# AnteMarusic/Accelerating-Genomics

Measured on AMD Instinct MI355X. Metric: Smith-Waterman affine-gap score-only GCUPS (config 2: 65536 pairs 150x150 per GPU), higher is better.
Workload: dtype int16x2 lanes, int32 scores; 1 GPU; BASELINE config 2: 65536 SW pairs 150x150 per GPU, iid ACGT + 25% related, newline sentinel aligned as the reference does; pairs_per_gpu=65536, len=150, cells_counted_per_pair=22500, parallelism=pairs sharded per GPU, no collective

## Files before the change

accelerating-genomics_amd/api.py:

```python
from __future__ import annotations

import ctypes as C
import os
import subprocess

import numpy as np

_HERE = os.path.dirname(os.path.abspath(__file__))
TUNING_KNOBS = ("AGX_SW_KERNEL", "AGX_SW_TAIL_BETA", "AGX_SW_MAX_C", "AGX_SW_FORCE_C", "AGX_SW_MAX_CLASSES", "AGX_SW_WAVES_PER_CLASS",
                "AGX_SW_SORT_WAVES", "AGX_SW_ONE_LAUNCH", "AGX_SW_DNA", "AGX_SW_RISE", "AGX_PHMM_PLAIN_CELL", "AGX_TRACE_CREATE", "AGX_HOST_THREADS", "AGX_FANOUT", "AGX_PHMM_TAB_BUDGET", "AGX_PHMM_MAX_C",
                "AGX_PHMM_FORCE_C", "AGX_PHMM_TAIL_BETA", "AGX_PHMM_MAX_CLASSES", "AGX_PHMM_NO_LUT", "AGX_TRACE_POOL", "AGX_NO_STREAM_PRIO", "AGX_SW_I32_CLASSIC", "AGX_SW_PIECE_MB", "AGX_SW_PIECE_MIN_PAIRS", "AGX_PHMM_NO_ROWS", "AGX_PHMM_NO_TRAINS", "AGX_PHMM_LUT_ONE_LOOP", "AGX_SW_HOST_PLAN", "AGX_PHMM_NO_RING")
_DEFAULT_LIB = "libagx_tuning.so" if any(k in os.environ for k in TUNING_KNOBS) else "libagx.so"
LIB_PATH = os.environ.get("AGX_LIB_PATH", os.path.join(_HERE, _DEFAULT_LIB))

OK, E_ARG, E_NODEVICE, E_HIP, E_NOMEM, E_SYMBOL, E_LIMIT, E_IO = 0, -1, -2, -3, -4, -5, -6, -7
OPT_SW_KERNEL = 1
OPT_SW_PLANNER = 2
SW_PLANNER_AUTO, SW_PLANNER_HOST, SW_PLANNER_DEVICE = 0, 1, 2
OPT_PHMM_TRAINS = 3
PHMM_TRAINS_AUTO, PHMM_TRAINS_OFF, PHMM_TRAINS_ON = 0, 1, 2
SW_KERNEL_AUTO, SW_KERNEL_INT32, SW_KERNEL_PACKED_SIGNED, SW_KERNEL_PACKED_BIASED = 0, 1, 2, 3
PHMM_F64, PHMM_F64_FMA, PHMM_F32, PHMM_F32_FMA = 0, 1, 2, 3
PHMM_GATK_PRIOR = 0x100

SYMBOLS = [
    "agx_version", "agx_last_error", "agx_device_count", "agx_device_name", "agx_ctx_create", "agx_ctx_destroy", "agx_ctx_device",
    "agx_ctx_stream", "agx_ctx_set_stream", "agx_ctx_sync", "agx_ctx_set_option", "agx_warmup_devices", "agx_host_alloc", "agx_host_free",
    "agx_ctx_timer_start", "agx_ctx_timer_stop", "agx_ctx_timer_mark", "agx_ctx_timer_elapsed",
    "agx_sw_batch_create", "agx_sw_batch_create_scored", "agx_sw_batch_create_matrix", "agx_sw_batch_launch", "agx_sw_batch_scores", "agx_sw_batch_bind_scores", "agx_sw_batch_info", "agx_sw_batch_destroy",
    "agx_sw_score", "agx_sw_score_multi", "agx_sw_score_devices", "agx_sw_shard_cuts",
    "agx_phmm_batch_create", "agx_phmm_batch_launch", "agx_phmm_batch_results", "agx_phmm_batch_bind_results", "agx_phmm_batch_info",
    "agx_phmm_batch_destroy", "agx_phmm_forward", "agx_phmm_forward_multi", "agx_phmm_forward_devices", "agx_phmm_shard_cuts",
    "agx_pairHMM",
    "agx_sw_text_read", "agx_sw_text_free", "agx_sw_reader_open", "agx_sw_reader_line_num", "agx_sw_reader_set_threads", "agx_sw_reader_next",
# ... 438 lines not shown
```

accelerating-genomics_amd/csrc/agx_sw.cpp:

```cpp
#include "agx_sw.h"

#include <algorithm>
#include <cmath>
#include <memory>
#include <mutex>
#include <thread>

#include "agx_internal.h"
#include "agx_parallel.h"

namespace {

struct Tiling {
    int cls;
    int G;
};

bool positive(long n) { return n > 0; }
bool at_least_4(long n) { return n >= 4; }
inline double tail_beta_override() { static const double v = agx_knob_real(agx_tune("AGX_SW_TAIL_BETA"), -1.0); return v; }
int max_cols_per_lane() { static const int v = (int)agx_knob_int(agx_tune("AGX_SW_MAX_C"), AGX_SW_MAX_COLS_PER_LANE, at_least_4); return v; }
int force_cols_per_lane() { static const int v = (int)agx_knob_int(agx_tune("AGX_SW_FORCE_C"), 0); return v; }
int max_classes_override() { static const int v = (int)agx_knob_int(agx_tune("AGX_SW_MAX_CLASSES"), 0, positive); return v; }
int tuned_kernel()
// ... 118 lines not shown
            best_cost = c;
        }
    }
    return best;
}

inline uint64_t piece_bytes() { static const uint64_t v = (uint64_t)agx_knob_int(agx_tune("AGX_SW_PIECE_MB"), 32, positive) << 20; return v; }
inline int64_t piece_min_pairs() { static const int64_t v = agx_knob_int(agx_tune("AGX_SW_PIECE_MIN_PAIRS"), 32768, positive); return v; }
constexpr size_t kRawPad = 64;
constexpr uint8_t kClsEmpty = 255;
constexpr uint8_t kClsUntiled = 254;
struct PairPlan {
    uint32_t pair;
    uint32_t ly;
    uint16_t lxo;
    uint8_t cls;
    uint8_t G;
    uint32_t lx() const { return lxo & 0x7fffu; }
};

struct ClassLaunch {
    int C = 0;
    uint32_t first_wave = 0, n_waves = 0;
};

struct Bucket {
    size_t first = 0, count = 0;
    size_t group0 = 0, n_groups = 0;
    size_t wave0 = 0, n_waves = 0;
    int cls = 0, G = 0;
};

}

struct agx_sw_batch {
    agx_ctx *ctx = nullptr;
    int family = 0;
    SwParams prm{};
    int64_t n_pairs = 0;
    DevBuf img, groups, waves, scores;
    DevBuf table;
    int rising = 0;
    PinBuf out_stage;
    bool matrix = false;
    std::vector<ClassLaunch> launches;
    agx_sw_info info{};
    struct SwPending *pending = nullptr;
// ... 903 lines not shown
        const char *e = agx_tune("AGX_SW_SORT_WAVES");
        return !(e && e[0] == '0');
    }();
    static const bool one_launch_ok = [] {
        const char *e = agx_tune("AGX_SW_ONE_LAUNCH");
        return !(e && e[0] == '0');
    }();
    if (family >= 2 && launches.size() > 1 && one_launch_ok) {
        if (sort_waves)
            std::stable_sort(waves.begin(), waves.end(), [](const SwWave &a, const SwWave &b) {
                return (uint64_t)a.steps * a.reserved > (uint64_t)b.steps * b.reserved;
            });
        ClassLaunch all_classes;
        all_classes.C = 0;
        all_classes.first_wave = 0;
        all_classes.n_waves = (uint32_t)waves.size();
        launches.assign(1, all_classes);
    } else if (sort_waves && !launches.empty())
        agx_pool_run((int)launches.size(), [&](int k) {
            const ClassLaunch &cl = launches[(size_t)k];
            std::stable_sort(waves.begin() + cl.first_wave, waves.begin() + cl.first_wave + cl.n_waves,
                             [](const SwWave &a, const SwWave &b) { return a.steps > b.steps; });
        });
    std::vector<uint32_t> x_dw(plan.size()), y_dw(plan.size());
    img_dw = img0;
    {
        const int parts = (int)std::min<int64_t>(agx_host_threads(), std::max<int64_t>(1, (int64_t)plan.size() / 16384));
        std::vector<size_t> part_sum((size_t)parts + 1, 0);
        const size_t chunk = (plan.size() + parts - 1) / (size_t)parts;
        auto words = [&](const PairPlan &pp, size_t *xw) {
            *xw = ((size_t)pp.G * kSwClasses[pp.cls] + 3) / 4 + 1;
            return *xw + ((size_t)pp.ly + 3) / 4;
        };
        agx_pool_run(parts, [&](int t) {
            const size_t lo = std::min(plan.size(), (size_t)t * chunk), hi = std::min(plan.size(), lo + chunk);
            size_t s = 0, xw;
            for (size_t i = lo; i < hi; ++i) s += words(plan[i], &xw);
            part_sum[(size_t)t + 1] = s;
        });
        for (int t = 0; t < parts; ++t) part_sum[(size_t)t + 1] += part_sum[(size_t)t];
        img_dw = img0 + part_sum[(size_t)parts];
        if (img_dw > 0xffffffffull) {
            agx_set_error("packed image exceeds 16 GiB; split the batch");
            return AGX_E_LIMIT;
        }
        agx_pool_run(parts, [&](int t) {
// ... 132 lines not shown
        agx_set_error("agx_sw_batch_create: upload -> %s", hipGetErrorString(e));
        return AGX_E_HIP;
    }
    if (device_plan) b->info.padded_cells = (int64_t) * (const unsigned long long *)dp.h_padded.p;
    if (flag[0]) {
        if (matrix)
            agx_set_error("pair %u contains a byte outside the substitution matrix's alphabet", flag[1]);
        else
            agx_set_error("pair %u contains byte 0x00, which is reserved as the padding symbol", flag[1]);
        return AGX_E_SYMBOL;
    }
    if (trace)
        fprintf(stderr,
                "[agx_sw_batch_create] %lld pairs%s: pass A %.2f ms | tiling %.2f, sort %.2f, waves %.2f, records %.2f | waited %.2f ms more "
                "for the upload of %.1f MB | device pack + sync %.2f ms\n",
                (long long)n_pairs, device_plan ? " (planned on the device)" : "", t_pass_a - t_begin, t_plan - t_pass_a, t_sort - t_plan, t_waves - t_sort, t_records - t_waves,
                t_joined - t_records, raw_bytes / 1e6, agx_now_ms() - t_joined);
    *out = b;
    b = nullptr;
    done.ok = true;
    return AGX_OK;
}

}

extern "C" {

int agx_sw_batch_launch(agx_sw_batch *b)
{
    if (!b) {
        agx_set_error("agx_sw_batch_launch: null batch");
        return AGX_E_ARG;
    }
    if (!b->ctx) {
        agx_set_error("this batch was planned without a context (no device): it cannot be launched");
        return AGX_E_NODEVICE;
    }
    int rc = agx_bind(b->ctx);
    if (rc) return rc;
    if (b->pending && b->pending->ready) AGX_HIP(hipStreamWaitEvent(b->ctx->stream, b->pending->ready, 0));
    SwParams prm = b->prm;
    if (b->bound) prm.n_out = (uint32_t)b->n_pairs;
    FanOut fan(b->ctx, (int)b->launches.size());
    rc = fan.begin();
    if (rc) return rc;
    int k = 0;
    for (auto it = b->launches.rbegin(); it != b->launches.rend(); ++it) {
        const ClassLaunch &cl = *it;
        hipStream_t st = fan.stream(k++);
        const uint32_t *img = (const uint32_t *)b->img.p;
        const SwWave *wv = (const SwWave *)b->waves.p + cl.first_wave;
        int32_t *scores = b->bound ? b->bound : (int32_t *)b->scores.p;
        int r;
        if (b->matrix)
            r = agx_sw_mat_launch_class(cl.C, prm, img, (const SwGroup *)b->groups.p, wv, cl.n_waves, scores,
                                        (const int16_t *)b->table.p, st);
        else if (b->family == 3)
            r = cl.C == 0 ? agx_sw_i32d_launch_any(prm, img, (const SwGroup2 *)b->groups.p, wv, cl.n_waves, scores, st)
                          : agx_sw_i32d_launch_class(cl.C, prm, img, (const SwGroup2 *)b->groups.p, wv, cl.n_waves, scores, st);
        else if (b->family == 2 && cl.C == 0)
            r = agx_sw_pk2_launch_any(b->rising, prm, img, (const SwGroup2 *)b->groups.p, wv, cl.n_waves, scores, st);
        else if (b->family == 2)
            r = agx_sw_pk2_launch_class(cl.C, b->rising, prm, img, (const SwGroup2 *)b->groups.p, wv, cl.n_waves, scores, st);
        else if (b->family == 1)
            r = agx_sw_pk_launch_class(cl.C, prm, img, (const SwGroup2 *)b->groups.p, wv, cl.n_waves, scores, st);
        else
            r = (cl.C > 40 ? agx_sw_wide_launch_class : agx_sw_launch_class)(cl.C, prm, img, (const SwGroup *)b->groups.p, wv,
                                                                             cl.n_waves, scores, st);
        if (r) {
            agx_set_error("sw_fill<%d> launch failed: %s", cl.C, hipGetErrorString(hipGetLastError()));
            return AGX_E_HIP;
        }
    }
    return fan.end();
}

int agx_sw_batch_scores(agx_sw_batch *b, int32_t *scores)
{
    if (!b || (!scores && b->n_pairs)) {
        agx_set_error("agx_sw_batch_scores: null argument");
        return AGX_E_ARG;
    }
    if (!b->ctx) {
        agx_set_error("this batch was planned without a context (no device): it has no scores");
        return AGX_E_NODEVICE;
    }
    int rc = agx_bind(b->ctx);
    if (rc) return rc;
    if (b->pending) {
        rc = finish_create(b);
        if (rc) return rc;
    }
    if (b->n_pairs == 0) {
        AGX_HIP(hipStreamSynchronize(b->ctx->stream));
        return AGX_OK;
    }
    const size_t bytes = (size_t)b->n_pairs * sizeof(int32_t);
    if (b->bound && scores == b->bound) {
        AGX_HIP(hipStreamSynchronize(b->ctx->stream));
        return AGX_OK;
    }
// ... 145 lines not shown
```

accelerating-genomics_amd/csrc/agx_sw.h:

```cpp
#pragma once
#include <hip/hip_runtime.h>

#include <algorithm>
#include <cstdint>

struct SwGroup {
    uint32_t x_dw;
    uint32_t y_dw;
    uint32_t lx_ly;
    uint32_t out;
};

struct SwParams {
    int32_t ge;
    int32_t gf;
    int32_t hd;
    int32_t delta;
    int32_t shift;
    uint32_t ge2, gf2, hd2, delta2;
    uint32_t age2, agf2, bias2;
    uint32_t n_out;
};

struct SwGroup2 {
    uint32_t x_dw[2];
    uint32_t y_dw[2];
    uint32_t lx_ly[2];
    uint32_t out[2];
};

struct SwWave {
    uint32_t first_group;
    uint16_t n_groups;
    uint16_t G;
    uint32_t steps;
    uint32_t reserved;
};

#define AGX_SW_FOR_EACH_CLASS(X) \
    X(4) X(6) X(8) X(10) X(12) X(14) X(16) X(18) X(20) X(22) X(24) X(26) X(28) X(30) X(32) X(34) X(36) X(38) X(40)
#define AGX_SW_FOR_EACH_WIDE_CLASS(X) X(80) X(120) X(160)
static const int kSwClasses[] = {4, 6, 8, 10, 12, 14, 16, 18, 20, 22, 24, 26, 28, 30, 32, 34, 36, 38, 40, 80, 120, 160};
static const int kSwPackedMaxShort = 64 * 40;
static const int kSwNumClasses = sizeof(kSwClasses) / sizeof(kSwClasses[0]);
static const double kSwClassCost[] = {1.373, 1.250, 1.178, 1.138, 1.112, 1.080, 1.051, 1.033, 1.025, 1.022, 1.014, 1.014, 1.011, 1.007, 1.007, 1.004, 1.004, 1.004, 1.000, 1.6, 2.2, 4.0};
static const double kSwPkClassCost[] = {1.543, 1.358, 1.278, 1.210, 1.173, 1.136, 1.111, 1.086, 1.068, 1.037, 1.025, 1.025, 1.019, 1.012, 1.006, 1.006, 1.006, 1.000, 1.000, 0, 0, 0};
static const double kSwPk2ClassCost[] = {1.851, 1.581, 1.450, 1.367, 1.318, 1.263, 1.196, 1.184, 1.145, 1.097, 1.095, 1.056, 1.049, 1.053, 1.025, 1.023, 1.022, 1.016, 1.000, 0, 0, 0};

static const double kSwI32dClassCost[] = {1.373, 1.250, 1.178, 1.138, 1.112, 1.080, 1.051, 1.033, 1.025, 1.022, 1.014, 1.014, 1.011, 1.007, 1.007, 1.004, 1.004, 1.004, 1.000, 0, 0, 0};

constexpr int kSwMatDim = 33;
int agx_sw_mat_launch_class(int cols_per_lane, const SwParams &prm, const uint32_t *img, const SwGroup *groups,
                            const SwWave *waves, uint32_t n_waves, int32_t *scores, const int16_t *table, hipStream_t s);
int agx_sw_pack_launch(bool matrix, int slots, const uint8_t *raw, const uint64_t *off, uint64_t base, const void *groups,
                       uint32_t n_groups, uint32_t n_pairs, uint32_t *img, const uint8_t *code, uint32_t *flag, int n_cu,
                       hipStream_t s);
int agx_sw_pack_dna_launch(const uint8_t *raw, const uint64_t *off, uint64_t base, void *groups, void *waves, uint32_t n_waves,
                           uint32_t n_pairs, uint32_t *img, uint32_t *flag, int n_cu, hipStream_t s);
int agx_sw_pk_launch_class(int cols_per_lane, const SwParams &prm, const uint32_t *img, const SwGroup2 *groups,
                           const SwWave *waves, uint32_t n_waves, int32_t *scores, hipStream_t s);
int agx_sw_pk2_launch_class(int cols_per_lane, int rising, const SwParams &prm, const uint32_t *img, const SwGroup2 *groups,
                            const SwWave *waves, uint32_t n_waves, int32_t *scores, hipStream_t s);
void agx_sw_pk2_preload();
void agx_sw_pack_preload();
void agx_sw_i32_preload();
int agx_sw_pk2_launch_any(int rising, const SwParams &prm, const uint32_t *img, const SwGroup2 *groups, const SwWave *waves, uint32_t n_waves,
                          int32_t *scores, hipStream_t s);
int agx_sw_i32d_launch_any(const SwParams &prm, const uint32_t *img, const SwGroup2 *groups, const SwWave *waves, uint32_t n_waves, int32_t *scores,
                           hipStream_t s);
int agx_sw_i32d_launch_class(int cols_per_lane, const SwParams &prm, const uint32_t *img, const SwGroup2 *groups, const SwWave *waves,
                             uint32_t n_waves, int32_t *scores, hipStream_t s);
void agx_sw_i32d_preload();
int agx_sw_launch_class(int cols_per_lane, const SwParams &prm, const uint32_t *img, const SwGroup *groups,
                        const SwWave *waves, uint32_t n_waves, int32_t *scores, hipStream_t s);
int agx_sw_wide_launch_class(int cols_per_lane, const SwParams &prm, const uint32_t *img, const SwGroup *groups,
                             const SwWave *waves, uint32_t n_waves, int32_t *scores, hipStream_t s);

constexpr uint32_t kSwPlanEmptyKey = 1u << 27;
constexpr uint32_t kSwPlanWaveKeyMax = (1u << 24) - 1u;
constexpr int kSwPlanBuckets = kSwNumClasses * 64;
struct SwPlanArgs {
    const uint32_t *len;
    uint32_t n_pairs, n_fill;
    const uint32_t *seg_first;
    const uint32_t *segs;
// ... 18 lines not shown
```

accelerating-genomics_amd/csrc/agx_sw_pk2_kernel.hip:

```cpp
#include "agx_sw.h"
#include <type_traits>

namespace {

typedef unsigned short u16x2 __attribute__((ext_vector_type(2)));

__device__ __forceinline__ u16x2 as_v(uint32_t v) { return __builtin_bit_cast(u16x2, v); }
__device__ __forceinline__ uint32_t as_u(u16x2 v) { return __builtin_bit_cast(uint32_t, v); }
__device__ __forceinline__ uint32_t umax2(uint32_t a, uint32_t b) { return as_u(__builtin_elementwise_max(as_v(a), as_v(b))); }
__device__ __forceinline__ uint32_t umin2(uint32_t a, uint32_t b) { return as_u(__builtin_elementwise_min(as_v(a), as_v(b))); }
typedef _Float16 f16x2 __attribute__((ext_vector_type(2)));
__device__ __forceinline__ uint32_t umax3(uint32_t a, uint32_t b, uint32_t c)
{
    const f16x2 x = __builtin_bit_cast(f16x2, a), y = __builtin_bit_cast(f16x2, b), z = __builtin_bit_cast(f16x2, c);
    return __builtin_bit_cast(uint32_t, __builtin_elementwise_maximum(__builtin_elementwise_maximum(x, y), z));
}
__device__ __forceinline__ uint32_t in_vgpr(uint32_t s)
{
    uint32_t r;
    asm volatile("v_mov_b32 %0, %1" : "=v"(r) : "s"(s));
    return r;
}

#define AGX_DPP_TAKE " wave_shr:1 row_mask:0xf bank_mask:0xf bound_ctrl:0\n"

#define AGX_FAST_HEAD(BYTE)                                                                                                  \
    asm("v_lshrrev_b32_sdwa %4, %6, %8 dst_sel:DWORD dst_unused:UNUSED_PAD src0_sel:" BYTE " src1_sel:DWORD\n"               \
        "v_lshrrev_b32_sdwa %5, %7, %8 dst_sel:DWORD dst_unused:UNUSED_PAD src0_sel:" BYTE " src1_sel:DWORD\n"               \
        "s_mov_b64 vcc, %9\n"                                                                                                \
        "v_cndmask_b32_dpp %0, %10, %12, vcc" AGX_DPP_TAKE "v_cndmask_b32_dpp %1, %11, %12, vcc" AGX_DPP_TAKE                \
        "v_cndmask_b32_dpp %2, %2, %4, vcc" AGX_DPP_TAKE "v_cndmask_b32_dpp %3, %3, %5, vcc" AGX_DPP_TAKE                    \
        : "=&v"(zl), "=&v"(fl), "+v"(ta), "+v"(tb), "=&v"(ma), "=&v"(mb)                                                     \
        : "v"(rowsA), "v"(rowsB), "v"(kv), "s"(start_mask), "v"(z_last), "v"(f_last), "v"(z0v)                               \
        : "vcc")

template <int K>
__device__ __forceinline__ void fast_head(uint32_t &zl, uint32_t &fl, uint32_t &ta, uint32_t &tb, uint32_t rowsA, uint32_t rowsB,
                                          uint32_t kv, uint64_t start_mask, uint32_t z_last, uint32_t f_last, uint32_t z0v)
{
    uint32_t ma, mb;
    if constexpr (K == 1)
        AGX_FAST_HEAD("BYTE_1");
    else if constexpr (K == 2)
        AGX_FAST_HEAD("BYTE_2");
    else if constexpr (K == 3)
        AGX_FAST_HEAD("BYTE_3");
    else
        AGX_FAST_HEAD("BYTE_0");
}

__device__ __forceinline__ void bytes_head(uint32_t &zl, uint32_t &fl, uint32_t &yc, uint32_t rowsA, uint32_t rowsB, uint32_t sel,
                                           uint32_t sh_sym, uint64_t start_mask, uint32_t z_last, uint32_t f_last, uint32_t z0v)
{
    uint32_t fresh;
    asm("v_perm_b32 %3, %5, %4, %6\n"
        "v_lshlrev_b32 %3, %7, %3\n"
        "s_mov_b64 vcc, %8\n"
        "v_cndmask_b32_dpp %0, %9, %11, vcc" AGX_DPP_TAKE "v_cndmask_b32_dpp %1, %10, %11, vcc" AGX_DPP_TAKE
        "v_cndmask_b32_dpp %2, %2, %3, vcc" AGX_DPP_TAKE
        : "=&v"(zl), "=&v"(fl), "+v"(yc), "=&v"(fresh)
        : "v"(rowsA), "v"(rowsB), "s"(sel), "v"(sh_sym), "s"(start_mask), "v"(z_last), "v"(f_last), "v"(z0v)
        : "vcc");
}

template <int C, bool FAST, int KC>
__device__ __forceinline__ void pk2_fill(const SwParams &prm, const uint32_t *__restrict__ img, const SwGroup2 &g, const SwWave &w,
                                         int32_t *__restrict__ scores, int lane, int G, int gl, bool active, bool start, bool feeder)
{
    constexpr int XW = (C + 3) / 4;
    constexpr bool RISE = KC > 0;
    constexpr int NK = KC > 1 ? KC : 1;
    constexpr int kEnd = KC > 1 ? (C - 1) % KC : 0;
    constexpr int NM = KC > 1 ? KC + 3 : NK;
    const uint32_t sh_sym = prm.shift;
    const uint32_t col_pad = 0x100u << sh_sym;
    const uint32_t ge = in_vgpr(prm.age2), gf = in_vgpr(RISE ? prm.agf2 - prm.age2 : prm.agf2);
    const uint32_t hd = in_vgpr(FAST ? prm.hd2 - prm.delta2 : prm.hd2);
    const uint32_t bias = prm.bias2, delta = prm.delta2;
    const uint32_t z0 = prm.bias2 - prm.agf2;
    const uint32_t hd0 = in_vgpr((FAST ? prm.hd2 - prm.delta2 : prm.hd2) + (RISE ? prm.age2 : 0u));
    const uint32_t hdw = in_vgpr((FAST ? prm.hd2 - prm.delta2 : prm.hd2) + prm.age2 - (uint32_t)NK * prm.age2);
    const uint32_t ge_wrap = in_vgpr((uint32_t)NK * prm.age2), c_end = in_vgpr((uint32_t)kEnd * prm.age2);
    const uint32_t hdf = KC > 1 && kEnd > 0 ? in_vgpr((FAST ? prm.hd2 - prm.delta2 : prm.hd2) + prm.age2 - (uint32_t)kEnd * prm.age2) : hd0;
    const uint32_t ge4 = in_vgpr(4u * prm.age2);
    uint32_t zb = (RISE ? z0 + prm.age2 : z0) + (uint32_t)kEnd * prm.age2;
    uint32_t floorv[NK];
#pragma unroll
    for (int k = 0; k < NK; ++k) floorv[k] = (RISE ? bias + prm.age2 : bias) + (uint32_t)k * prm.age2;
    const uint32_t z_init = RISE ? z0 + prm.age2 : z0;
    const uint32_t kv = in_vgpr((prm.delta2 & 0xffu) << 24);
    const uint64_t start_mask = __ballot(start);
    const uint32_t lx_mask = FAST ? 0xfffu : 0x7fffu;
    const int lxA = (int)(g.lx_ly[0] & lx_mask), lxB = (int)(g.lx_ly[1] & lx_mask);
    const int lyA = (int)(g.lx_ly[0] >> 16), lyB = (int)(g.lx_ly[1] >> 16);

    const uint32_t no_row = FAST ? 0x1f1f1f1fu : 0u;
    const uint32_t *ybA = lyA > 0 ? img + g.y_dw[0] : img, *ybB = lyB > 0 ? img + g.y_dw[1] : img;
    const uint32_t lastA = lyA > 0 ? (uint32_t)((lyA + 3) >> 2) - 1u : 0u, lastB = lyB > 0 ? (uint32_t)((lyB + 3) >> 2) - 1u : 0u;
    const int nqA = feeder ? (lyA + 3) >> 2 : 0, nqB = feeder ? (lyB + 3) >> 2 : 0;
    auto loadA = [&](int q) -> uint32_t { return ybA[min((uint32_t)q, lastA)]; };
    auto loadB = [&](int q) -> uint32_t { return ybB[min((uint32_t)q, lastB)]; };
    auto row_selA = [&](int q, uint32_t v) -> uint32_t { return q < nqA ? v : no_row; };
    auto row_selB = [&](int q, uint32_t v) -> uint32_t { return q < nqB ? v : no_row; };

    uint32_t xq[C];
    constexpr int PF = C < 8 ? 2 : 1;
    uint32_t nextA[PF], nextB[PF];
    {
        const uint32_t o = (uint32_t)gl * C, d0 = o >> 2, sh = o & 3u;
        const uint32_t fillA = (FAST && !(active && g.x_dw[0])) ? 0x0c0c0c0cu : 0u;
        const uint32_t fillB = (FAST && !(active && g.x_dw[1])) ? 0x0c0c0c0cu : 0u;
        uint32_t ra[XW + 1], rb[XW + 1];
#pragma unroll
        for (int k = 0; k <= XW; ++k) {
            ra[k] = img[g.x_dw[0] + d0 + k];
            rb[k] = img[g.x_dw[1] + d0 + k];
        }
#pragma unroll
        for (int r = 0; r < PF; ++r) {
            nextA[r] = loadA(r);
            nextB[r] = loadB(r);
        }
        __builtin_amdgcn_s_waitcnt(0x0f70);
        __builtin_amdgcn_sched_barrier(0);
#pragma unroll
        for (int k = 0; k <= XW; ++k) {
            ra[k] |= fillA;
            rb[k] |= fillB;
        }
#pragma unroll
        for (int k = 0; k < XW; ++k) {
            const uint32_t a = __builtin_amdgcn_alignbyte(ra[k + 1], ra[k], sh);
            const uint32_t b = __builtin_amdgcn_alignbyte(rb[k + 1], rb[k], sh);
#pragma unroll
            for (int i = 0; i < 4; ++i)
                if (4 * k + i < C) {
                    const uint32_t ca = (a >> (8 * i)) & 0xffu, cb = (b >> (8 * i)) & 0xffu;
                    uint32_t v;
                    if constexpr (FAST)
                        v = ca | 0x0c00u | (cb << 16) | 0x0c000000u;
                    else {
                        const int col = (int)o + 4 * k + i;
                        v = (col < lxA ? ca << sh_sym : col_pad) | ((col < lxB ? cb << sh_sym : col_pad) << 16);
                    }
                    asm volatile("" : "+v"(v));
                    xq[4 * k + i] = v;
                }
        }
    }

    uint32_t z[C], e[C];
#pragma unroll
    for (int j = 0; j < C; ++j) {
        z[j] = z_init + (uint32_t)(j % NK) * prm.age2;
        e[j] = bias + (uint32_t)(j % NK) * prm.age2;
    }
    uint32_t z_last = z_init + (uint32_t)kEnd * prm.age2, f_last = z_last, diag_in = z0 + (uint32_t)kEnd * prm.age2;
    uint32_t best[NM];
#pragma unroll
    for (int k = 0; k < NM; ++k) best[k] = z_init + (uint32_t)(KC > 1 ? k + 1 : k) * prm.age2;
    uint32_t yc = 0;
    uint32_t ta = 0, tb = 0;

    const bool last = active && gl == G - 1;
    const bool nlA = FAST && last && ((g.lx_ly[0] >> 13) & 1u), nlB = FAST && last && ((g.lx_ly[1] >> 13) & 1u);
    const int capA_t = (nlA && lxA > 0 && lyA > 0) ? lyA + G - 2 : -1, capB_t = (nlB && lxB > 0 && lyB > 0) ? lyB + G - 2 : -1;
    uint32_t cornerA = z_init + (uint32_t)kEnd * prm.age2, cornerB = cornerA;

    const int steps = (int)w.steps;
    uint32_t rowsA = 0, rowsB = 0;
    int t = 0;

    auto take_max = [&](auto sc) __attribute__((always_inline)) {
        constexpr int S = decltype(sc)::value;
#pragma unroll
        for (int k = 0; k < NK; ++k) {
#pragma unroll
            for (int j = k; j < C; j += 2 * NK) {
                if (j + NK < C)
                    best[S + k] = umax3(best[S + k], z[j], z[j + NK]);
                else
                    best[S + k] = umax2(best[S + k], z[j]);
            }
        }
    };

    auto step = [&](auto kc, auto sc, auto cc) __attribute__((always_inline)) {
        constexpr int K = decltype(kc)::value;
        constexpr int S = decltype(sc)::value;
        constexpr bool CAP = decltype(cc)::value;
// ... 56 lines not shown
        ++t;
    };

    auto rise4 = [&]() __attribute__((always_inline)) {
        if constexpr (KC > 1) {
#pragma unroll
            for (int m = 0; m < NM; ++m) best[m] += ge4;
        }
    };
    auto quad_of_steps = [&](auto cc) __attribute__((always_inline)) {
        step(std::integral_constant<int, 0>{}, std::integral_constant<int, 0>{}, cc);
        step(std::integral_constant<int, 1>{}, std::integral_constant<int, 1>{}, cc);
        step(std::integral_constant<int, 2>{}, std::integral_constant<int, 2>{}, cc);
        step(std::integral_constant<int, 3>{}, std::integral_constant<int, 3>{}, cc);
        rise4();
    };
    auto take = [&](int q, int r) __attribute__((always_inline)) {
        rowsA = row_selA(q, nextA[r]);
        rowsB = row_selB(q, nextB[r]);
        nextA[r] = loadA(q + PF);
        nextB[r] = loadB(q + PF);
    };
    const int quads = steps >> 2;
    int cap_first = 0x7fffffff;
    if constexpr (FAST) {
        cap_first = min(capA_t < 0 ? 0x7fffffff : capA_t, capB_t < 0 ? 0x7fffffff : capB_t);
        for (int o = 32; o > 0; o >>= 1) cap_first = min(cap_first, __shfl_xor(cap_first, o));
        cap_first = __builtin_amdgcn_readfirstlane(cap_first);
    }
    const int quads_free = min(quads, cap_first >> 2);
    constexpr std::integral_constant<bool, false> no_cap{};
    constexpr std::integral_constant<bool, FAST> cap{};
    int q = 0;
    if constexpr (PF == 1) {
        if constexpr (FAST) {
            for (; q < quads_free; ++q) {
                take(q, 0);
                quad_of_steps(no_cap);
            }
        }
        for (; q < quads; ++q) {
            take(q, 0);
            quad_of_steps(cap);
        }
    } else {
        if constexpr (FAST) {
            for (; q + 1 < quads_free; q += 2) {
                take(q, 0);
                quad_of_steps(no_cap);
                take(q + 1, 1);
                quad_of_steps(no_cap);
            }
// ... 7 lines not shown
        if (q < quads) {
            rowsA = row_selA(q, nextA[0]);
            rowsB = row_selB(q, nextB[0]);
            quad_of_steps(cap);
            ++q;
            nextA[0] = nextA[1];
            nextB[0] = nextB[1];
        }
    }
    rowsA = row_selA(q, nextA[0]);
    rowsB = row_selB(q, nextB[0]);
#pragma unroll 1
    while (t < steps) {
        step(std::integral_constant<int, 0>{}, std::integral_constant<int, 4>{}, cap);
        rowsA >>= 8;
        rowsB >>= 8;
        if constexpr (KC > 1) {
            const uint32_t b0 = best[0];
#pragma unroll
            for (int m = 0; m + 1 < NM; ++m) best[m] = best[m + 1];
            best[NM - 1] = b0 + (uint32_t)NM * prm.age2;
        }
    }
    if constexpr (KC > 1) {
#pragma unroll
        for (int m = 0; m + 1 < NM; ++m) best[NM - 1] = umax2(best[NM - 1], best[m] + (uint32_t)(NM - 1 - m) * prm.age2);
        best[0] = best[NM - 1] - (uint32_t)NM * prm.age2;
    }

    if constexpr (FAST) {
        const uint32_t match2 = prm.hd2 - prm.agf2;
        const uint32_t ge1 = RISE ? prm.age2 & 0xffffu : 0u;
        const uint32_t off_end = (uint32_t)kEnd * (prm.age2 & 0xffffu);
        uint32_t cand = best[0];
        if (nlA) cand = (cand & 0xffff0000u) | ((cornerA + match2 + (uint32_t)(steps - 1 - capA_t) * ge1 - off_end) & 0xffffu);
        if (nlB) cand = (cand & 0xffffu) | ((cornerB + match2 + (((uint32_t)(steps - 1 - capB_t) * ge1 - off_end) << 16)) & 0xffff0000u);
        best[0] = umax2(best[0], cand);
    }
    uint32_t bestv = best[0];
    for (int o = 1; o < G; o <<= 1) {
        const uint32_t other = (uint32_t)__shfl_down((int)bestv, o);
        if (gl + o < G) bestv = umax2(bestv, other);
    }
    {
        const int off = (int)(z0 & 0xffffu) + (RISE ? (steps + 1) * (int)(prm.age2 & 0xffffu) : 0);
        const int src = (lane * G) & 63;
        const int sa = __shfl((int)(bestv & 0xffffu) - off, src), sb = __shfl((int)(bestv >> 16) - off, src);
        const uint32_t oa = (uint32_t)__shfl((int)g.out[0], src), ob = (uint32_t)__shfl((int)g.out[1], src);
        if (lane < (int)w.n_groups) {
            if (ob == oa + 1u && !(oa & 1u) && ob < prm.n_out)
                *reinterpret_cast<int2 *>(scores + oa) = make_int2(sa, sb);
            else {
                scores[oa] = sa;
                if (ob < prm.n_out) scores[ob] = sb;
            }
        }
    }
}

template <int C, int KC>
__device__ __forceinline__ void pk2_body(const SwParams &prm, const uint32_t *__restrict__ img, const SwGroup2 *__restrict__ groups,
                                         const SwWave w, int32_t *__restrict__ scores)
{
    static_assert(C % 2 == 0, "the running maximum takes two columns per instruction");
    constexpr int KCC = KC > 1 && C < 14 ? 1 : KC;
    const int lane = threadIdx.x & 63;
    const int G = w.G;
    const int grp = lane / G;
    const int gl = lane - grp * G;
    const bool active = grp < (int)w.n_groups;
    const bool start = gl == 0;
    const bool feeder = active && start;

    SwGroup2 g = groups[w.first_group + (active ? grp : 0)];
    __builtin_amdgcn_s_waitcnt(0x0f70);
    __builtin_amdgcn_sched_barrier(0);
#pragma unroll
    for (int k = 0; k < 2; ++k) {
        g.x_dw[k] = active ? g.x_dw[k] : 0u;
        g.y_dw[k] = active ? g.y_dw[k] : 0u;
        g.lx_ly[k] = active ? g.lx_ly[k] : 0u;
        g.out[k] = active ? g.out[k] : 0u;
    }
    if (__builtin_amdgcn_readfirstlane(w.reserved >> 16) & 1u)
        pk2_fill<C, true, KCC>(prm, img, g, w, scores, lane, G, gl, active, start, feeder);
    else
        pk2_fill<C, false, KCC>(prm, img, g, w, scores, lane, G, gl, active, start, feeder);
}

template <int C, int KC>
__global__ void __launch_bounds__(256) sw_fill_pk2(const SwParams prm, const uint32_t *__restrict__ img,
                                                   const SwGroup2 *__restrict__ groups,
                                                   const SwWave *__restrict__ waves, uint32_t n_waves,
                                                   int32_t *__restrict__ scores)
{
    const uint32_t wave = __builtin_amdgcn_readfirstlane(blockIdx.x * 4u + (threadIdx.x >> 6));
    if (wave >= n_waves) return;
    pk2_body<C, KC>(prm, img, groups, waves[wave], scores);
}

template <int KC>
__global__ void __launch_bounds__(256) sw_fill_pk2_any(const SwParams prm, const uint32_t *__restrict__ img,
                                                       const SwGroup2 *__restrict__ groups,
                                                       const SwWave *__restrict__ waves, uint32_t n_waves,
                                                       int32_t *__restrict__ scores)
{
    const uint32_t wave = __builtin_amdgcn_readfirstlane(blockIdx.x * 4u + (threadIdx.x >> 6));
    if (wave >= n_waves) return;
    const SwWave w = waves[wave];
    switch (__builtin_amdgcn_readfirstlane(w.reserved) & 0xffffu) {
#define AGX_SW_CASE(CC) \
    case CC: pk2_body<CC, KC>(prm, img, groups, w, scores); break;
        AGX_SW_FOR_EACH_CLASS(AGX_SW_CASE)
#undef AGX_SW_CASE
    default: break;
    }
}

template <int C, int KC>
int launch(const SwParams &prm, const uint32_t *img, const SwGroup2 *groups, const SwWave *waves, uint32_t n_waves,
           int32_t *scores, hipStream_t s)
{
    const uint32_t blocks = (n_waves + 3) / 4;
    hipLaunchKernelGGL((sw_fill_pk2<C, KC>), dim3(blocks), dim3(256), 0, s, prm, img, groups, waves, n_waves, scores);
    return hipGetLastError() == hipSuccess ? 0 : -1;
}

}

int agx_sw_pk2_launch_any(int rising, const SwParams &prm, const uint32_t *img, const SwGroup2 *groups, const SwWave *waves, uint32_t n_waves,
                          int32_t *scores, hipStream_t s)
{
    if (n_waves == 0) return 0;
    const uint32_t blocks = (n_waves + 3) / 4;
    if (rising == 4)
        hipLaunchKernelGGL(sw_fill_pk2_any<4>, dim3(blocks), dim3(256), 0, s, prm, img, groups, waves, n_waves, scores);
    else if (rising)
        hipLaunchKernelGGL(sw_fill_pk2_any<1>, dim3(blocks), dim3(256), 0, s, prm, img, groups, waves, n_waves, scores);
    else
        hipLaunchKernelGGL(sw_fill_pk2_any<0>, dim3(blocks), dim3(256), 0, s, prm, img, groups, waves, n_waves, scores);
    return hipGetLastError() == hipSuccess ? 0 : -1;
}

int agx_sw_pk2_launch_class(int cols_per_lane, int rising, const SwParams &prm, const uint32_t *img, const SwGroup2 *groups,
                            const SwWave *waves, uint32_t n_waves, int32_t *scores, hipStream_t s)
{
    if (n_waves == 0) return 0;
    switch (cols_per_lane) {
#define AGX_SW_CASE(CC) \
    case CC: return rising == 4 ? launch<CC, 4>(prm, img, groups, waves, n_waves, scores, s) : rising ? launch<CC, 1>(prm, img, groups, waves, n_waves, scores, s) : launch<CC, 0>(prm, img, groups, waves, n_waves, scores, s);
        AGX_SW_FOR_EACH_CLASS(AGX_SW_CASE)
#undef AGX_SW_CASE
    default: return -2;
    }
}

void agx_sw_pk2_preload()
{
    hipFuncAttributes a;
    (void)hipFuncGetAttributes(&a, reinterpret_cast<const void *>(&sw_fill_pk2_any<4>));
}
```

Before: 8992 GCUPS.

## Compute group index directly for uniform wave layouts and overlap setup with loads

The host now detects per-class wave lists where groups are laid out contiguously with a fixed G, and passes that shape through SwParams so the per-class kernel can compute its group record address without first loading the wave descriptor. This removes one dependent global load from the kernel prologue. The fill prologue is reordered so register initialisation, the sequence loads and the cap reduction overlap with the outstanding group-record load. Cross-lane reductions switch to DPP sequences, and query packing uses a byte-permute instead of masks and shifts. A timestamp-instrumented kernel variant is added behind an opt-in knob for profiling.

```diff
diff --git a/accelerating-genomics_amd/api.py b/accelerating-genomics_amd/api.py
--- a/accelerating-genomics_amd/api.py
+++ b/accelerating-genomics_amd/api.py
@@ -9,7 +9,7 @@
 _HERE = os.path.dirname(os.path.abspath(__file__))
 TUNING_KNOBS = ("AGX_SW_KERNEL", "AGX_SW_TAIL_BETA", "AGX_SW_MAX_C", "AGX_SW_FORCE_C", "AGX_SW_MAX_CLASSES", "AGX_SW_WAVES_PER_CLASS",
                 "AGX_SW_SORT_WAVES", "AGX_SW_ONE_LAUNCH", "AGX_SW_DNA", "AGX_SW_RISE", "AGX_PHMM_PLAIN_CELL", "AGX_TRACE_CREATE", "AGX_HOST_THREADS", "AGX_FANOUT", "AGX_PHMM_TAB_BUDGET", "AGX_PHMM_MAX_C",
-                "AGX_PHMM_FORCE_C", "AGX_PHMM_TAIL_BETA", "AGX_PHMM_MAX_CLASSES", "AGX_PHMM_NO_LUT", "AGX_TRACE_POOL", "AGX_NO_STREAM_PRIO", "AGX_SW_I32_CLASSIC", "AGX_SW_PIECE_MB", "AGX_SW_PIECE_MIN_PAIRS", "AGX_PHMM_NO_ROWS", "AGX_PHMM_NO_TRAINS", "AGX_PHMM_LUT_ONE_LOOP", "AGX_SW_HOST_PLAN", "AGX_PHMM_NO_RING")
+                "AGX_PHMM_FORCE_C", "AGX_PHMM_TAIL_BETA", "AGX_PHMM_MAX_CLASSES", "AGX_PHMM_NO_LUT", "AGX_TRACE_POOL", "AGX_NO_STREAM_PRIO", "AGX_SW_I32_CLASSIC", "AGX_SW_PIECE_MB", "AGX_SW_PIECE_MIN_PAIRS", "AGX_PHMM_NO_ROWS", "AGX_PHMM_NO_TRAINS", "AGX_PHMM_LUT_ONE_LOOP", "AGX_SW_HOST_PLAN", "AGX_PHMM_NO_RING", "AGX_SW_STAMPS", "AGX_SW_STAMPS_FILE")
 _DEFAULT_LIB = "libagx_tuning.so" if any(k in os.environ for k in TUNING_KNOBS) else "libagx.so"
 LIB_PATH = os.environ.get("AGX_LIB_PATH", os.path.join(_HERE, _DEFAULT_LIB))
 
diff --git a/accelerating-genomics_amd/csrc/agx_sw.cpp b/accelerating-genomics_amd/csrc/agx_sw.cpp
--- a/accelerating-genomics_amd/csrc/agx_sw.cpp
+++ b/accelerating-genomics_amd/csrc/agx_sw.cpp
@@ -164,7 +164,24 @@
 struct ClassLaunch {
     int C = 0;
     uint32_t first_wave = 0, n_waves = 0;
+    uint32_t uni_shape = 0, uni_group0 = 0, uni_last = 0;
 };
+
+void mark_uniform(ClassLaunch &cl, const std::vector<SwWave> &waves)
+{
+    cl.uni_shape = cl.uni_group0 = cl.uni_last = 0;
+    if (cl.C == 0 || cl.n_waves == 0) return;
+    const SwWave *w = waves.data() + cl.first_wave;
+    const uint32_t G = w[0].G, per_wave = G ? 64u / G : 0u, n = cl.n_waves;
+    if (!per_wave) return;
+    for (uint32_t i = 0; i < n; ++i) {
+        if (w[i].G != G || w[i].first_group != w[0].first_group + i * per_wave) return;
+        if (w[i].n_groups == 0 || w[i].n_groups > per_wave || (i + 1 < n && w[i].n_groups != per_wave)) return;
+    }
+    cl.uni_shape = G | per_wave << 16;
+    cl.uni_group0 = w[0].first_group;
+    cl.uni_last = w[n - 1].first_group + w[n - 1].n_groups - 1u;
+}
 
 struct Bucket {
     size_t first = 0, count = 0;
@@ -1114,6 +1131,8 @@
             std::stable_sort(waves.begin() + cl.first_wave, waves.begin() + cl.first_wave + cl.n_waves,
                              [](const SwWave &a, const SwWave &b) { return a.steps > b.steps; });
         });
+    if (family == 2)
+        for (ClassLaunch &cl : launches) mark_uniform(cl, waves);
     std::vector<uint32_t> x_dw(plan.size()), y_dw(plan.size());
     img_dw = img0;
     {
@@ -1292,12 +1311,69 @@
     return AGX_OK;
 }
 
+bool stamps_wanted()
+{
+    static const bool v = agx_knob_int(agx_tune("AGX_SW_STAMPS"), 0) != 0;
+    return v;
+}
+struct StampRun {
+    void *dev = nullptr;
+    uint32_t cap = 0, n_waves = 0;
+    double host_ms[4] = {0, 0, 0, 0};
+};
+StampRun &stamp_run()
+{
+    static StampRun r;
+    return r;
+}
+int launch_stamped(agx_ctx *, const SwParams &prm, const uint32_t *img, const SwGroup2 *groups, const SwWave *waves, uint32_t n_waves,
+                   int32_t *scores, hipStream_t s)
+{
+    StampRun &r = stamp_run();
+    if (n_waves > r.cap) {
+        if (r.dev) (void)hipFree(r.dev);
+        r.dev = nullptr;
+        r.cap = 0;
+        if (hipMalloc(&r.dev, (size_t)n_waves * kSwStampBytes) != hipSuccess) return -1;
+        r.cap = n_waves;
+    }
+    r.n_waves = n_waves;
+    return agx_sw_pk2_launch_stamped(prm, img, groups, waves, n_waves, scores, r.dev, s);
+}
+void write_stamps()
+{
+    StampRun &r = stamp_run();
+    const char *path = agx_tune("AGX_SW_STAMPS_FILE");
+    if (!r.n_waves || !path) return;
+    std::vector<uint8_t> h((size_t)r.n_waves * kSwStampBytes);
+    if (hipMemcpy(h.data(), r.dev, h.size(), hipMemcpyDeviceToHost) != hipSuccess) return;
+    if (FILE *f = fopen(path, "ab")) {
+        const uint32_t head[2] = {r.n_waves, 0};
+        fwrite(head, sizeof(head), 1, f);
+        fwrite(r.host_ms, sizeof(r.host_ms), 1, f);
+        fwrite(h.data(), 1, h.size(), f);
+        fclose(f);
+    }
+    r.n_waves = 0;
+}
+struct StampClock {
+    int at;
+    explicit StampClock(int a) : at(a) { if (stamps_wanted()) stamp_run().host_ms[at] = agx_now_ms(); }
+    ~StampClock()
+    {
+        if (!stamps_wanted()) return;
+        stamp_run().host_ms[at + 1] = agx_now_ms();
+        if (at == 2) write_stamps();
+    }
+};
+
 }
 
 extern "C" {
 
 int agx_sw_batch_launch(agx_sw_batch *b)
 {
+    StampClock stamp_clock(0);
     if (!b) {
         agx_set_error("agx_sw_batch_launch: null batch");
         return AGX_E_ARG;
@@ -1330,8 +1406,16 @@
                           : agx_sw_i32d_launch_class(cl.C, prm, img, (const SwGroup2 *)b->groups.p, wv, cl.n_waves, scores, st);
         else if (b->family == 2 && cl.C == 0)
             r = agx_sw_pk2_launch_any(b->rising, prm, img, (const SwGroup2 *)b->groups.p, wv, cl.n_waves, scores, st);
-        else if (b->family == 2)
-            r = agx_sw_pk2_launch_class(cl.C, b->rising, prm, img, (const SwGroup2 *)b->groups.p, wv, cl.n_waves, scores, st);
+        else if (b->family == 2) {
+            SwParams up = prm;
+            up.uni_shape = cl.uni_shape;
+            up.uni_group0 = cl.uni_group0;
+            up.uni_last = cl.uni_last;
+            if (stamps_wanted() && cl.C == 38 && b->rising == 4)
+                r = launch_stamped(b->ctx, up, img, (const SwGroup2 *)b->groups.p, wv, cl.n_waves, scores, st);
+            else
+                r = agx_sw_pk2_launch_class(cl.C, b->rising, up, img, (const SwGroup2 *)b->groups.p, wv, cl.n_waves, scores, st);
+        }
         else if (b->family == 1)
             r = agx_sw_pk_launch_class(cl.C, prm, img, (const SwGroup2 *)b->groups.p, wv, cl.n_waves, scores, st);
         else
@@ -1347,6 +1431,7 @@
 
 int agx_sw_batch_scores(agx_sw_batch *b, int32_t *scores)
 {
+    StampClock stamp_clock(2);
     if (!b || (!scores && b->n_pairs)) {
         agx_set_error("agx_sw_batch_scores: null argument");
         return AGX_E_ARG;
diff --git a/accelerating-genomics_amd/csrc/agx_sw.h b/accelerating-genomics_amd/csrc/agx_sw.h
--- a/accelerating-genomics_amd/csrc/agx_sw.h
+++ b/accelerating-genomics_amd/csrc/agx_sw.h
@@ -20,6 +20,7 @@
     uint32_t ge2, gf2, hd2, delta2;
     uint32_t age2, agf2, bias2;
     uint32_t n_out;
+    uint32_t uni_shape, uni_group0, uni_last;
 };
 
 struct SwGroup2 {
@@ -61,6 +62,9 @@
                            const SwWave *waves, uint32_t n_waves, int32_t *scores, hipStream_t s);
 int agx_sw_pk2_launch_class(int cols_per_lane, int rising, const SwParams &prm, const uint32_t *img, const SwGroup2 *groups,
                             const SwWave *waves, uint32_t n_waves, int32_t *scores, hipStream_t s);
+constexpr size_t kSwStampBytes = 48;
+int agx_sw_pk2_launch_stamped(const SwParams &prm, const uint32_t *img, const SwGroup2 *groups, const SwWave *waves, uint32_t n_waves,
+                              int32_t *scores, void *stamps, hipStream_t s);
 void agx_sw_pk2_preload();
 void agx_sw_pack_preload();
 void agx_sw_i32_preload();
diff --git a/accelerating-genomics_amd/csrc/agx_sw_pk2_kernel.hip b/accelerating-genomics_amd/csrc/agx_sw_pk2_kernel.hip
--- a/accelerating-genomics_amd/csrc/agx_sw_pk2_kernel.hip
+++ b/accelerating-genomics_amd/csrc/agx_sw_pk2_kernel.hip
@@ -21,6 +21,31 @@
     asm volatile("v_mov_b32 %0, %1" : "=v"(r) : "s"(s));
     return r;
 }
+
+template <int CTRL>
+__device__ __forceinline__ uint32_t dpp_take(uint32_t v)
+{
+    return (uint32_t)__builtin_amdgcn_update_dpp((int)v, (int)v, CTRL, 0xf, 0xf, false);
+}
+constexpr int kDppXor1 = 0xb1, kDppXor2 = 0x4e, kDppHalfMirror = 0x141, kDppMirror = 0x140;
+
+__device__ __forceinline__ int wave_min(int v)
+{
+    v = min(v, (int)dpp_take<kDppXor1>((uint32_t)v));
+    v = min(v, (int)dpp_take<kDppXor2>((uint32_t)v));
+    v = min(v, (int)dpp_take<kDppHalfMirror>((uint32_t)v));
+    v = min(v, (int)dpp_take<kDppMirror>((uint32_t)v));
+    return min(min(__builtin_amdgcn_readlane(v, 0), __builtin_amdgcn_readlane(v, 16)),
+               min(__builtin_amdgcn_readlane(v, 32), __builtin_amdgcn_readlane(v, 48)));
+}
+
+struct SwStamps {
+    uint64_t t[4];
+    uint32_t hw_id;
+    uint32_t xcc_id;
+    uint32_t pad[2];
+};
+static_assert(sizeof(SwStamps) == 48, "tools/sw_step_budget.py reads 48-byte records");
 
 #define AGX_DPP_TAKE " wave_shr:1 row_mask:0xf bank_mask:0xf bound_ctrl:0\n"
 
@@ -63,10 +88,18 @@
         : "vcc");
 }
 
-template <int C, bool FAST, int KC>
-__device__ __forceinline__ void pk2_fill(const SwParams &prm, const uint32_t *__restrict__ img, const SwGroup2 &g, const SwWave &w,
-                                         int32_t *__restrict__ scores, int lane, int G, int gl, bool active, bool start, bool feeder)
-{
+template <int C, bool FAST, int KC, bool STAMP>
+__device__ __forceinline__ void pk2_fill(const SwParams &prm, const uint32_t *__restrict__ img, SwGroup2 &g, const SwWave &w,
+                                         int32_t *__restrict__ scores, int lane, int G, int gl, bool active, bool start, bool feeder,
+                                         SwStamps *__restrict__ stamp, uint64_t t_entry)
+{
+    auto wait_record = [&]() __attribute__((always_inline)) {
+        __builtin_amdgcn_s_waitcnt(0x0f70);
+        __builtin_amdgcn_sched_barrier(0);
+        asm volatile("" : "+v"(g.x_dw[0]), "+v"(g.x_dw[1]), "+v"(g.y_dw[0]), "+v"(g.y_dw[1]), "+v"(g.lx_ly[0]), "+v"(g.lx_ly[1]),
+                     "+v"(g.out[0]), "+v"(g.out[1]));
+    };
+    if constexpr (!FAST) wait_record();
     constexpr int XW = (C + 3) / 4;
     constexpr bool RISE = KC > 0;
     constexpr int NK = KC > 1 ? KC : 1;
@@ -90,6 +123,31 @@
     const uint32_t z_init = RISE ? z0 + prm.age2 : z0;
     const uint32_t kv = in_vgpr((prm.delta2 & 0xffu) << 24);
     const uint64_t start_mask = __ballot(start);
+
+    uint32_t z[C], e[C];
+#pragma unroll
+    for (int j = 0; j < C; ++j) {
+        z[j] = in_vgpr(z_init + (uint32_t)(j % NK) * prm.age2);
+        e[j] = in_vgpr(bias + (uint32_t)(j % NK) * prm.age2);
+    }
+    uint32_t z_last = in_vgpr(z_init + (uint32_t)kEnd * prm.age2), f_last = z_last, diag_in = in_vgpr(z0 + (uint32_t)kEnd * prm.age2);
+    uint32_t best[NM];
+#pragma unroll
+    for (int k = 0; k < NM; ++k) best[k] = in_vgpr(z_init + (uint32_t)(KC > 1 ? k + 1 : k) * prm.age2);
+    uint32_t yc = 0;
+    uint32_t ta = 0, tb = 0;
+
+    uint32_t cornerA = z_last, cornerB = cornerA;
+
+
+    if constexpr (FAST) wait_record();
+#pragma unroll
+    for (int k = 0; k < 2; ++k) {
+        g.x_dw[k] = active ? g.x_dw[k] : 0u;
+        g.y_dw[k] = active ? g.y_dw[k] : 0u;
+        g.lx_ly[k] = active ? g.lx_ly[k] : 0u;
+        g.out[k] = active ? g.out[k] : 0u;
+    }
     const uint32_t lx_mask = FAST ? 0xfffu : 0x7fffu;
     const int lxA = (int)(g.lx_ly[0] & lx_mask), lxB = (int)(g.lx_ly[1] & lx_mask);
     const int lyA = (int)(g.lx_ly[0] >> 16), lyB = (int)(g.lx_ly[1] >> 16);
@@ -106,66 +164,50 @@
     uint32_t xq[C];
     constexpr int PF = C < 8 ? 2 : 1;
     uint32_t nextA[PF], nextB[PF];
-    {
-        const uint32_t o = (uint32_t)gl * C, d0 = o >> 2, sh = o & 3u;
-        const uint32_t fillA = (FAST && !(active && g.x_dw[0])) ? 0x0c0c0c0cu : 0u;
-        const uint32_t fillB = (FAST && !(active && g.x_dw[1])) ? 0x0c0c0c0cu : 0u;
-        uint32_t ra[XW + 1], rb[XW + 1];
-#pragma unroll
-        for (int k = 0; k <= XW; ++k) {
-            ra[k] = img[g.x_dw[0] + d0 + k];
-            rb[k] = img[g.x_dw[1] + d0 + k];
-        }
-#pragma unroll
-        for (int r = 0; r < PF; ++r) {
-            nextA[r] = loadA(r);
-            nextB[r] = loadB(r);
-        }
-        __builtin_amdgcn_s_waitcnt(0x0f70);
-        __builtin_amdgcn_sched_barrier(0);
-#pragma unroll
-        for (int k = 0; k <= XW; ++k) {
-            ra[k] |= fillA;
-            rb[k] |= fillB;
-        }
-#pragma unroll
-        for (int k = 0; k < XW; ++k) {
-            const uint32_t a = __builtin_amdgcn_alignbyte(ra[k + 1], ra[k], sh);
-            const uint32_t b = __builtin_amdgcn_alignbyte(rb[k + 1], rb[k], sh);
-#pragma unroll
-            for (int i = 0; i < 4; ++i)
-                if (4 * k + i < C) {
-                    const uint32_t ca = (a >> (8 * i)) & 0xffu, cb = (b >> (8 * i)) & 0xffu;
-                    uint32_t v;
-                    if constexpr (FAST)
-                        v = ca | 0x0c00u | (cb << 16) | 0x0c000000u;
-                    else {
-                        const int col = (int)o + 4 * k + i;
-                        v = (col < lxA ? ca << sh_sym : col_pad) | ((col < lxB ? cb << sh_sym : col_pad) << 16);
-                    }
-                    asm volatile("" : "+v"(v));
-                    xq[4 * k + i] = v;
-                }
-        }
-    }
-
-    uint32_t z[C], e[C];
-#pragma unroll
-    for (int j = 0; j < C; ++j) {
-        z[j] = z_init + (uint32_t)(j % NK) * prm.age2;
-        e[j] = bias + (uint32_t)(j % NK) * prm.age2;
-    }
-    uint32_t z_last = z_init + (uint32_t)kEnd * prm.age2, f_last = z_last, diag_in = z0 + (uint32_t)kEnd * prm.age2;
-    uint32_t best[NM];
-#pragma unroll
-    for (int k = 0; k < NM; ++k) best[k] = z_init + (uint32_t)(KC > 1 ? k + 1 : k) * prm.age2;
-    uint32_t yc = 0;
-    uint32_t ta = 0, tb = 0;
+    const uint32_t o = (uint32_t)gl * C, d0 = o >> 2, sh = o & 3u;
+    const bool vacantA = FAST && !(active && g.x_dw[0]), vacantB = FAST && !(active && g.x_dw[1]);
+    uint32_t ra[XW + 1], rb[XW + 1];
+#pragma unroll
+    for (int k = 0; k <= XW; ++k) {
+        ra[k] = img[g.x_dw[0] + d0 + k];
+        rb[k] = img[g.x_dw[1] + d0 + k];
+    }
+#pragma unroll
+    for (int r = 0; r < PF; ++r) {
+        nextA[r] = loadA(r);
+        nextB[r] = loadB(r);
+    }
 
     const bool last = active && gl == G - 1;
     const bool nlA = FAST && last && ((g.lx_ly[0] >> 13) & 1u), nlB = FAST && last && ((g.lx_ly[1] >> 13) & 1u);
     const int capA_t = (nlA && lxA > 0 && lyA > 0) ? lyA + G - 2 : -1, capB_t = (nlB && lxB > 0 && lyB > 0) ? lyB + G - 2 : -1;
-    uint32_t cornerA = z_init + (uint32_t)kEnd * prm.age2, cornerB = cornerA;
+    int cap_first = 0x7fffffff;
+    if constexpr (FAST) cap_first = wave_min(min(capA_t < 0 ? 0x7fffffff : capA_t, capB_t < 0 ? 0x7fffffff : capB_t));
+    const uint32_t sel_or = 0x0c000c00u | (vacantA ? 0x0cu : 0u) | (vacantB ? 0x0c0000u : 0u);
+
+    __builtin_amdgcn_s_waitcnt(0x0f70);
+    __builtin_amdgcn_sched_barrier(0);
+#pragma unroll
+    for (int k = 0; k < XW; ++k) {
+        const uint32_t a = __builtin_amdgcn_alignbyte(ra[k + 1], ra[k], sh);
+        const uint32_t b = __builtin_amdgcn_alignbyte(rb[k + 1], rb[k], sh);
+#pragma unroll
+        for (int i = 0; i < 4; ++i)
+            if (4 * k + i < C) {
+                uint32_t v;
+                if constexpr (FAST)
+                    v = __builtin_amdgcn_perm(b, a, 0x0c000c00u + (uint32_t)i * 0x00010001u + 0x00040000u) | sel_or;
+                else {
+                    const uint32_t ca = (a >> (8 * i)) & 0xffu, cb = (b >> (8 * i)) & 0xffu;
+                    const int col = (int)o + 4 * k + i;
+                    v = (col < lxA ? ca << sh_sym : col_pad) | ((col < lxB ? cb << sh_sym : col_pad) << 16);
+                }
+                asm volatile("" : "+v"(v));
+                xq[4 * k + i] = v;
+            }
+    }
+    uint64_t t_first = 0, t_loop = 0;
+    if constexpr (STAMP) t_first = __builtin_amdgcn_s_memrealtime();
 
     const int steps = (int)w.steps;
     uint32_t rowsA = 0, rowsB = 0;
@@ -268,12 +310,6 @@
         nextB[r] = loadB(q + PF);
     };
     const int quads = steps >> 2;
-    int cap_first = 0x7fffffff;
-    if constexpr (FAST) {
-        cap_first = min(capA_t < 0 ? 0x7fffffff : capA_t, capB_t < 0 ? 0x7fffffff : capB_t);
-        for (int o = 32; o > 0; o >>= 1) cap_first = min(cap_first, __shfl_xor(cap_first, o));
-        cap_first = __builtin_amdgcn_readfirstlane(cap_first);
-    }
     const int quads_free = min(quads, cap_first >> 2);
     constexpr std::integral_constant<bool, false> no_cap{};
     constexpr std::integral_constant<bool, FAST> cap{};
@@ -327,6 +363,7 @@
             best[NM - 1] = b0 + (uint32_t)NM * prm.age2;
         }
     }
+    if constexpr (STAMP) t_loop = __builtin_amdgcn_s_memrealtime();
     if constexpr (KC > 1) {
 #pragma unroll
         for (int m = 0; m + 1 < NM; ++m) best[NM - 1] = umax2(best[NM - 1], best[m] + (uint32_t)(NM - 1 - m) * prm.age2);
@@ -343,14 +380,22 @@
         best[0] = umax2(best[0], cand);
     }
     uint32_t bestv = best[0];
-    for (int o = 1; o < G; o <<= 1) {
-        const uint32_t other = (uint32_t)__shfl_down((int)bestv, o);
-        if (gl + o < G) bestv = umax2(bestv, other);
+    if (G <= 16 && !(G & (G - 1))) {
+        bestv = umax2(bestv, dpp_take<kDppXor1>(bestv) & (G >= 2 ? ~0u : 0u));
+        bestv = umax2(bestv, dpp_take<kDppXor2>(bestv) & (G >= 4 ? ~0u : 0u));
+        bestv = umax2(bestv, dpp_take<kDppHalfMirror>(bestv) & (G >= 8 ? ~0u : 0u));
+        bestv = umax2(bestv, dpp_take<kDppMirror>(bestv) & (G >= 16 ? ~0u : 0u));
+    } else {
+        for (int d = 1; d < G; d <<= 1) {
+            const uint32_t other = (uint32_t)__shfl_down((int)bestv, d);
+            if (gl + d < G) bestv = umax2(bestv, other);
+        }
     }
     {
         const int off = (int)(z0 & 0xffffu) + (RISE ? (steps + 1) * (int)(prm.age2 & 0xffffu) : 0);
         const int src = (lane * G) & 63;
-        const int sa = __shfl((int)(bestv & 0xffffu) - off, src), sb = __shfl((int)(bestv >> 16) - off, src);
+        const uint32_t both = (uint32_t)__shfl((int)bestv, src);
+        const int sa = (int)(both & 0xffffu) - off, sb = (int)(both >> 16) - off;
         const uint32_t oa = (uint32_t)__shfl((int)g.out[0], src), ob = (uint32_t)__shfl((int)g.out[1], src);
         if (lane < (int)w.n_groups) {
             if (ob == oa + 1u && !(oa & 1u) && ob < prm.n_out)
@@ -361,36 +406,46 @@
             }
         }
     }
-}
-
-template <int C, int KC>
+    if constexpr (STAMP) {
+        __builtin_amdgcn_s_waitcnt(0x0f70);
+        const uint64_t t_end = __builtin_amdgcn_s_memrealtime();
+        if (lane == 0) {
+            stamp->t[0] = t_entry;
+            stamp->t[1] = t_first;
+            stamp->t[2] = t_loop;
+            stamp->t[3] = t_end;
+            stamp->hw_id = __builtin_amdgcn_s_getreg(4 | (31 << 11));
+            stamp->xcc_id = __builtin_amdgcn_s_getreg(20 | (31 << 11));
+        }
+    }
+    asm volatile("; fill of %0 columns, DNA-coded %1, ends" ::"n"(C), "n"((int)FAST));
+}
+
+template <int C, int KC, bool UNI, bool STAMP>
 __device__ __forceinline__ void pk2_body(const SwParams &prm, const uint32_t *__restrict__ img, const SwGroup2 *__restrict__ groups,
-                                         const SwWave w, int32_t *__restrict__ scores)
+                                         const SwWave w, uint32_t wave, int32_t *__restrict__ scores, SwStamps *__restrict__ stamp,
+                                         uint64_t t_entry)
 {
     static_assert(C % 2 == 0, "the running maximum takes two columns per instruction");
     constexpr int KCC = KC > 1 && C < 14 ? 1 : KC;
     const int lane = threadIdx.x & 63;
-    const int G = w.G;
-    const int grp = lane / G;
+    const uint32_t shape = UNI ? prm.uni_shape : 0u;
+    int G = max((int)(shape & 0xffffu), 1), grp = lane / G;
+    SwGroup2 g;
+    if constexpr (UNI) g = groups[min(prm.uni_group0 + wave * (shape >> 16) + (uint32_t)grp, prm.uni_last)];
+    if (!shape) {
+        G = w.G;
+        grp = lane / G;
+        g = groups[w.first_group + (grp < (int)w.n_groups ? grp : 0)];
+    }
     const int gl = lane - grp * G;
     const bool active = grp < (int)w.n_groups;
     const bool start = gl == 0;
     const bool feeder = active && start;
-
-    SwGroup2 g = groups[w.first_group + (active ? grp : 0)];
-    __builtin_amdgcn_s_waitcnt(0x0f70);
-    __builtin_amdgcn_sched_barrier(0);
-#pragma unroll
-    for (int k = 0; k < 2; ++k) {
-        g.x_dw[k] = active ? g.x_dw[k] : 0u;
-        g.y_dw[k] = active ? g.y_dw[k] : 0u;
-        g.lx_ly[k] = active ? g.lx_ly[k] : 0u;
-        g.out[k] = active ? g.out[k] : 0u;
-    }
     if (__builtin_amdgcn_readfirstlane(w.reserved >> 16) & 1u)
-        pk2_fill<C, true, KCC>(prm, img, g, w, scores, lane, G, gl, active, start, feeder);
+        pk2_fill<C, true, KCC, STAMP>(prm, img, g, w, scores, lane, G, gl, active, start, feeder, stamp, t_entry);
     else
-        pk2_fill<C, false, KCC>(prm, img, g, w, scores, lane, G, gl, active, start, feeder);
+        pk2_fill<C, false, KCC, STAMP>(prm, img, g, w, scores, lane, G, gl, active, start, feeder, stamp, t_entry);
 }
 
 template <int C, int KC>
@@ -401,7 +456,19 @@
 {
     const uint32_t wave = __builtin_amdgcn_readfirstlane(blockIdx.x * 4u + (threadIdx.x >> 6));
     if (wave >= n_waves) return;
-    pk2_body<C, KC>(prm, img, groups, waves[wave], scores);
+    pk2_body<C, KC, true, false>(prm, img, groups, waves[wave], wave, scores, nullptr, 0);
+}
+
+template <int C, int KC>
+__global__ void __launch_bounds__(256) sw_fill_pk2_stamped(const SwParams prm, const uint32_t *__restrict__ img,
+                                                           const SwGroup2 *__restrict__ groups,
+                                                           const SwWave *__restrict__ waves, uint32_t n_waves,
+                                                           int32_t *__restrict__ scores, SwStamps *__restrict__ stamps)
+{
+    const uint64_t t_entry = __builtin_amdgcn_s_memrealtime();
+    const uint32_t wave = __builtin_amdgcn_readfirstlane(blockIdx.x * 4u + (threadIdx.x >> 6));
+    if (wave >= n_waves) return;
+    pk2_body<C, KC, true, true>(prm, img, groups, waves[wave], wave, scores, stamps + wave, t_entry);
 }
 
 template <int KC>
@@ -415,7 +482,7 @@
     const SwWave w = waves[wave];
     switch (__builtin_amdgcn_readfirstlane(w.reserved) & 0xffffu) {
 #define AGX_SW_CASE(CC) \
-    case CC: pk2_body<CC, KC>(prm, img, groups, w, scores); break;
+    case CC: pk2_body<CC, KC, false, false>(prm, img, groups, w, wave, scores, nullptr, 0); break;
         AGX_SW_FOR_EACH_CLASS(AGX_SW_CASE)
 #undef AGX_SW_CASE
     default: break;
@@ -447,6 +514,16 @@
     return hipGetLastError() == hipSuccess ? 0 : -1;
 }
 
+int agx_sw_pk2_launch_stamped(const SwParams &prm, const uint32_t *img, const SwGroup2 *groups, const SwWave *waves, uint32_t n_waves,
+                              int32_t *scores, void *stamps, hipStream_t s)
+{
+    static_assert(sizeof(SwStamps) == kSwStampBytes, "agx_sw.cpp sizes the stamp buffer by kSwStampBytes");
+    if (n_waves == 0) return 0;
+    hipLaunchKernelGGL((sw_fill_pk2_stamped<38, 4>), dim3((n_waves + 3) / 4), dim3(256), 0, s, prm, img, groups, waves, n_waves, scores,
+                       (SwStamps *)stamps);
+    return hipGetLastError() == hipSuccess ? 0 : -1;
+}
+
 int agx_sw_pk2_launch_class(int cols_per_lane, int rising, const SwParams &prm, const uint32_t *img, const SwGroup2 *groups,
                             const SwWave *waves, uint32_t n_waves, int32_t *scores, hipStream_t s)
 {
```

Result: no change. 9060 GCUPS (median of 6 runs) (+0.8%).
